# Diegotistical/OptionsLab

Hardware: AMD Instinct MI355X
Metric: MC path-steps/sec (1M paths × 252 steps Euro call); price vs BS |err|/σ (higher is better)
Workload: dtype f32 normals / f64 prices

## Files before the change

### include/olmc.h

```cpp
#ifndef OLMC_H
#define OLMC_H

#include <stdint.h>

#ifdef __cplusplus
extern "C" {
#endif

#define OLMC_ABI_VERSION 6

enum {
    OLMC_OK = 0,
    OLMC_ERR_ARG = 1,
    OLMC_ERR_HIP = 2,
    OLMC_ERR_STATE = 3,
    OLMC_ERR_RCCL = 4
};

enum { OLMC_STREAM_GBM = 0, OLMC_STREAM_HESTON = 1, OLMC_STREAM_JUMP = 2, OLMC_STREAM_KOU = 3 };
enum { OLMC_STREAM_HESTON_QE = 0x48514500 };
enum { OLMC_AVG_ARITHMETIC = 0, OLMC_AVG_GEOMETRIC = 1, OLMC_AVG_ARITHMETIC_FAST = 2 };
#define OLMC_MAX_BATCH 16

typedef struct olmc_stats {
// ... 239 lines not shown
                            const uint32_t* shift, int32_t bits, int antithetic, olmc_stats* out);

int olmc_multi_gpu_european(double S, double K, double T, double r, double sigma, double q, int is_call,
                            int64_t n_paths, int32_t n_steps, uint64_t seed, int antithetic,
                            int n_gpus, olmc_stats* out);
int olmc_multi_gpu_greeks_fd(double S, double K, double T, double r, double sigma, double q, int is_call,
                             int64_t n_paths, int32_t n_steps, uint64_t seed, int second_order,
                             int n_gpus, double* out9, olmc_stats* evals );
int olmc_multi_gpu_european_cv(double S, double K, double T, double r, double sigma, double q, int is_call,
                               int64_t n_paths, int32_t n_steps, uint64_t seed, int antithetic,
                               int n_gpus, olmc_cv_moments* out);
int olmc_multi_gpu_european_qmc(double S, double K, double T, double r, double sigma, double q, int is_call,
                                int64_t n_paths, int32_t dims, const uint32_t* sv, const uint32_t* shift, int32_t bits,
                                int n_gpus, olmc_stats* out);
int olmc_multi_gpu_european_qmc_greeks_fd(double S, double K, double T, double r, double sigma, double q, int is_call,
                                          int64_t n_paths, int32_t dims, const uint32_t* sv, const uint32_t* shift, int32_t bits,
                                          int second_order, int n_gpus, double* out9, olmc_stats* evals );
int olmc_multi_gpu_european_qmc_cv(double S, double K, double T, double r, double sigma, double q, int is_call,
                                   int64_t n_paths, int32_t dims, const uint32_t* sv, const uint32_t* shift, int32_t bits,
                                   int n_gpus, olmc_cv_moments* out);
int olmc_multi_gpu_spans(double* out8);

int olmc_fetch_dev(const double* d_src, int32_t n, void* hip_stream, double* out_host);

int olmc_combine_stats(const olmc_stats* parts, int32_t n_parts, double r, double T, olmc_stats* out);

int olmc_philox_words(uint64_t seed, int64_t path_offset, int64_t n_paths,
                      int32_t block0, int32_t n_blocks, uint32_t stream_tag, uint32_t* out_host);
int olmc_normals(uint64_t seed, int64_t path_offset, int64_t n_paths, int32_t n_steps,
                 float* out_host);

int olmc_profile_enable(int on);
enum { OLMC_TUNE_GRID_CAP = 2, OLMC_TUNE_QMC_BLOCK = 4, OLMC_TUNE_SPLIT_TAIL = 7, OLMC_TUNE_POLL = 8, OLMC_TUNE_SPLIT_SAT = 9,
       OLMC_TUNE_MULTI_LAUNCH = 10, OLMC_TUNE_STAGED_COPY = 11 };
int olmc_tune(int knob, int value);
int olmc_profile_reset(void);
int olmc_kernel_time(int64_t* launches, double* total_ms);

#ifdef __cplusplus
}
#endif
#endif
```

### optionslab_amd/csrc/olmc.hip

```cpp
#include "olmc.h"
#include "olmc_kernels.h"
#include "olmc_job_board.h"

#include <dlfcn.h>
#include <sched.h>
#include <time.h>
#include <hip/hip_ext.h>
#include <rccl/rccl.h>

#include <algorithm>
#include <atomic>
#include <chrono>
#include <climits>
#include <condition_variable>
#include <cmath>
#include <cstdio>
#include <cstdlib>
#include <cstring>
#include <functional>
#include <limits>
#include <mutex>
#include <string>
#include <system_error>
#include <thread>
// ... 26 lines not shown
constexpr int kMaxNV = 2 * OLMC_MAX_BATCH;
constexpr int32_t kMaxGrid = 1 << 18;
constexpr int32_t kMaxGroups = kMaxGrid / kGroupBlocks + 1;
static_assert(kMaxGroups * kMaxNV == kGroupRowsCapacity, "device-side guard must match the group_rows allocation");

struct EventPair {
    hipEvent_t start, stop;
};

struct DeviceCtx {
    int device = -1;
    int cus = 0;
    hipStream_t stream = nullptr;
    struct WsSlot {
        double* block_rows = nullptr;
        size_t cap = 0;
        double* group_rows = nullptr;
        uint32_t* counters = nullptr;
        hipEvent_t done = nullptr;
        bool used = false;
        bool claimed = false;
        hipStream_t owner = nullptr;
        bool shared = false;
    };
    static constexpr int kSlots = 8;
    WsSlot slots[kSlots + 1];
    int next_slot = 0, cur_slot = 0;
    uint64_t* h_flag = nullptr;
    uint64_t* d_flag = nullptr;
    uint64_t seq = 0;
    uint64_t armed = 0;
    double* h_result = nullptr;
    double* d_result = nullptr;
    void* d_bulk = nullptr;
    size_t bulk_bytes = 0;
    void* h_stage[2] = {nullptr, nullptr};
    hipEvent_t stage_landed[2] = {nullptr, nullptr};
    void* d_multi = nullptr;
    void* h_multi = nullptr;
    void* d_h_multi = nullptr;
    int64_t multi_cap = 0;
    size_t multi_bpo = 0;
    size_t multi_off_done = 0, multi_off_opts = 0, multi_off_rows = 0, multi_hoff_out = 0;
    uint32_t* d_sobol = nullptr;
    size_t sobol_words = 0;
    std::vector<uint32_t> sobol_host;
    void* d_bridge = nullptr;
    int32_t bridge_n = 0;
    std::vector<unsigned char> bridge_host;
    double* d_heston_w = nullptr;
    size_t heston_w_bytes = 0;
    bool busy = false;
    std::vector<EventPair> ev_free, ev_pending;
    int64_t prof_launches = 0;
    double prof_ms = 0.0;
};

constexpr int kMaxContexts = 8;

struct DevicePool {
    std::mutex mu;
    std::condition_variable idle;
    std::vector<DeviceCtx*> all;
    int device = -1;
};

std::mutex g_mu;
std::atomic<DevicePool*> g_pool[kMaxDevices] = {};
std::atomic<int> g_default_device{-1};
bool g_profile = false;

int ctx_allocate(DeviceCtx* c) {
    HIP_TRY(hipStreamCreateWithFlags(&c->stream, hipStreamNonBlocking));
    for (auto& sl : c->slots) {
        HIP_TRY(hipMalloc(&sl.group_rows, sizeof(double) * kMaxNV * kMaxGroups));
        HIP_TRY(hipMalloc(&sl.counters, sizeof(uint32_t) * (kMaxGroups + 1) * kCounterStride));
        HIP_TRY(hipMemset(sl.counters, 0, sizeof(uint32_t) * (kMaxGroups + 1) * kCounterStride));
        HIP_TRY(hipEventCreateWithFlags(&sl.done, hipEventDisableTiming));
    }
    HIP_TRY(hipHostMalloc(&c->h_result, sizeof(double) * (kMaxNV + 1 + 15), hipHostMallocMapped));
    HIP_TRY(hipHostGetDevicePointer(reinterpret_cast<void**>(&c->d_result), c->h_result, 0));
    c->h_flag = reinterpret_cast<uint64_t*>(c->h_result + kMaxNV + 8);
    c->d_flag = reinterpret_cast<uint64_t*>(c->d_result + kMaxNV + 8);
    *c->h_flag = 0;
    return OLMC_OK;
}

void ctx_release(DeviceCtx* c) {
    if (c->stream) (void)hipStreamSynchronize(c->stream);
    for (auto& ep : c->ev_pending) { (void)hipEventDestroy(ep.start); (void)hipEventDestroy(ep.stop); }
    for (auto& ep : c->ev_free) { (void)hipEventDestroy(ep.start); (void)hipEventDestroy(ep.stop); }
    if (c->d_bulk) (void)hipFree(c->d_bulk);
    for (int i = 0; i < 2; ++i) {
        if (c->h_stage[i]) (void)hipHostFree(c->h_stage[i]);
        if (c->stage_landed[i]) (void)hipEventDestroy(c->stage_landed[i]);
    }
    if (c->d_multi) (void)hipFree(c->d_multi);
    if (c->h_multi) (void)hipHostFree(c->h_multi);
    if (c->d_sobol) (void)hipFree(c->d_sobol);
    if (c->d_bridge) (void)hipFree(c->d_bridge);
    if (c->d_heston_w) (void)hipFree(c->d_heston_w);
    for (auto& sl : c->slots) {
        if (sl.block_rows) (void)hipFree(sl.block_rows);
        if (sl.group_rows) (void)hipFree(sl.group_rows);
        if (sl.counters) (void)hipFree(sl.counters);
        if (sl.done) (void)hipEventDestroy(sl.done);
    }
    if (c->h_result) (void)hipHostFree(c->h_result);
    if (c->stream) (void)hipStreamDestroy(c->stream);
    delete c;
}

int ctx_create(int device, DeviceCtx** out) {
    int count = 0;
    hipError_t e = hipGetDeviceCount(&count);
    if (e != hipSuccess || count <= 0)
        return fail(OLMC_ERR_HIP, std::string("no HIP device available: ") + hipGetErrorString(e));
    if (device < 0 || device >= count || device >= kMaxDevices)
        return fail(OLMC_ERR_ARG, "device index out of range");
    HIP_TRY(hipSetDevice(device));
    hipDeviceProp_t prop;
    HIP_TRY(hipGetDeviceProperties(&prop, device));
    DeviceCtx* c = new DeviceCtx();
    c->device = device;
    c->cus = prop.multiProcessorCount;
    const int rc = ctx_allocate(c);
    if (rc) {
        ctx_release(c);
        return rc;
    }
    *out = c;
    return OLMC_OK;
}

struct CtxLease {
    DeviceCtx* c = nullptr;
    DevicePool* pool = nullptr;
    CtxLease() = default;
    CtxLease(const CtxLease&) = delete;
    CtxLease& operator=(const CtxLease&) = delete;
    ~CtxLease() { release(); }
// ... 120 lines not shown
        if (err == hipSuccess) err = hipEventRecord(c->stage_landed[slot], c->stream);
        if (err == hipSuccess && i >= 1) {
            const auto t = clock::now();
            err = hipEventSynchronize(c->stage_landed[slot ^ 1]);
            if (i == 1) us_first = us_since(t); else us_events += us_since(t);
            if (err == hipSuccess) landed.store(i, std::memory_order_release);
        }
    }
    {
        const auto t = clock::now();
        if (err == hipSuccess) err = hipEventSynchronize(c->stage_landed[(n_chunks - 1) & 1]);
        us_events += us_since(t);
    }
    if (err == hipSuccess) landed.store(n_chunks, std::memory_order_release);
    else give_up.store(true);
    const auto t_join = clock::now();
    for (std::thread& t : threads) t.join();
    if (trace)
        std::fprintf(stderr, "[olmc copy_to_host] %.1f MB, %lld chunks, %d threads: spawn %.0f us, first chunk landed (kernel + DMA) %.0f us, later event waits %.0f us, "
                             "waits for the copy threads %.0f us, last chunk out + join %.0f us, total %.0f us\n", bytes / 1e6, static_cast<long long>(n_chunks), n_threads,
                     us_spawn, us_first, us_events, us_workers, us_since(t_join), us_since(t_begin));
    if (err != hipSuccess) {
        (void)hipStreamSynchronize(c->stream);
        (void)hipGetLastError();
        return fail(OLMC_ERR_HIP, std::string("copy_to_host: ") + hipGetErrorString(err));
    }
    return OLMC_OK;
}

int g_multi_launch = 0;
int g_grid_cap = 0;
int g_qmc_block = 0;
int g_poll = 0;
int g_split_tail = 0;
int g_split_sat = 0;
#ifdef OLMC_WITH_PROBES
int g_fault_shard = 0;
int g_force_nv = 0;
int g_multi_rehearsal = 0;
#endif

constexpr int32_t kShortPathSteps = 128, kShortPathGrid = 4096;

int32_t grid_for(int64_t n_paths, int32_t n_steps = INT32_MAX) {
    int64_t cap = g_grid_cap > 0 ? std::min<int64_t>(g_grid_cap, kMaxGrid) : kMaxGrid;
    if (g_grid_cap == 0 && n_steps <= kShortPathSteps) cap = kShortPathGrid;
    return static_cast<int32_t>(std::min<int64_t>((n_paths + kBlock - 1) / kBlock, cap));
}

template <typename Kernel>
int resident_workgroups(Kernel kernel) {
    static std::mutex mu;
    static std::vector<std::pair<const void*, int>> cache;
    const void* key = reinterpret_cast<const void*>(kernel);
    std::lock_guard<std::mutex> lock(mu);
    for (const auto& e : cache)
        if (e.first == key) return e.second;
    int nb = 0;
    if (hipOccupancyMaxActiveBlocksPerMultiprocessor(&nb, kernel, kBlock, 0) != hipSuccess || nb < 1) {
        (void)hipGetLastError();
        nb = 1;
    }
    cache.emplace_back(key, nb);
    return nb;
}

// ... 39 lines not shown
            if (!taken.shared) {
                HIP_TRY(hipDeviceSynchronize());
                taken.shared = true;
                taken.used = false;
            }
        }
    }
    DeviceCtx::WsSlot& sl = c->slots[idx];
    c->cur_slot = idx;
    const bool guarded = !own && sl.shared;
    const size_t need = static_cast<size_t>(grid) * nv;
    if (need > sl.cap) {
        if (!guarded) HIP_TRY(hipStreamSynchronize(stream));
        else if (sl.used) HIP_TRY(hipEventSynchronize(sl.done));
        if (sl.block_rows) HIP_TRY(hipFree(sl.block_rows));
        sl.block_rows = nullptr;
        sl.cap = 0;
        const size_t cap = std::max<size_t>(need, size_t(1) << 16);
        HIP_TRY(hipMalloc(&sl.block_rows, sizeof(double) * cap));
        sl.cap = cap;
    }
    if (guarded && sl.used) HIP_TRY(hipStreamWaitEvent(stream, sl.done, 0));
    ws->block_rows = sl.block_rows;
    ws->group_rows = sl.group_rows;
    ws->counters = sl.counters;
    ws->out = d_out;
    ws->tail = tail;
    ws->row_capacity = sl.cap;
#ifdef OLMC_WITH_PROBES
    if (g_force_nv > 0) ws->row_capacity = static_cast<uint64_t>(grid) * g_force_nv;
#endif
    ws->done_flag = nullptr;
    ws->done_value = 0;
    c->armed = 0;
    if (own && d_out == c->d_result && g_poll >= 0) {
        c->armed = ++c->seq;
        ws->done_flag = c->d_flag;
        ws->done_value = c->armed;
    }
    return OLMC_OK;
}

void ws_recover(DeviceCtx* c) {
    c->armed = 0;
    (void)hipDeviceSynchronize();
    (void)hipGetLastError();
    for (auto& sl : c->slots) (void)hipMemset(sl.counters, 0, sizeof(uint32_t) * (kMaxGroups + 1) * kCounterStride);
}

void multi_recover(DeviceCtx* c) {
    c->armed = 0;
    (void)hipDeviceSynchronize();
    (void)hipGetLastError();
    if (c->d_multi) (void)hipMemset(c->d_multi, 0, c->multi_off_opts);
}

int after_launch(DeviceCtx* c, hipStream_t stream) {
    hipError_t e = hipGetLastError();
    if (e != hipSuccess) { ws_recover(c); return fail(OLMC_ERR_HIP, std::string("kernel launch: ") + hipGetErrorString(e)); }
    if (c->cur_slot == DeviceCtx::kSlots || !c->slots[c->cur_slot].shared) return OLMC_OK;
    DeviceCtx::WsSlot& sl = c->slots[c->cur_slot];
    HIP_TRY(hipEventRecord(sl.done, stream));
    sl.used = true;
    return OLMC_OK;
}

int prof_begin(DeviceCtx* c, hipStream_t s, EventPair* ep) {
    if (c->ev_free.empty()) {
        HIP_TRY(hipEventCreate(&ep->start));
        HIP_TRY(hipEventCreate(&ep->stop));
    } else {
        *ep = c->ev_free.back();
        c->ev_free.pop_back();
    }
    HIP_TRY(hipEventRecord(ep->start, s));
    return OLMC_OK;
}
// ... 149 lines not shown
        };
        if (nsets == 1) {
            ContractSet<1> cs;
            cs.c[0] = make_contract(opts[0], n_steps);
            cs.base_mask = 1u; cs.upper_continues_slot0 = 0;
            if (pos) pos[0] = 0;
            launch_european<1, kReduce>(anti, g, st, pr, cs, ws, nullptr, timed);
        } else if (nsets == 8) {
            fused(std::integral_constant<int, 8>{});
        } else {
            fused(std::integral_constant<int, 16>{});
        }
    }, profiled);
}

constexpr int64_t kSpinUs = 200, kYieldUs = 2000, kSleepUs = 20;

struct TimerSlack {
    long old = -1;
    void tighten() {
        if (old >= 0) return;
        old = prctl(PR_GET_TIMERSLACK, 0, 0, 0, 0);
        if (old >= 0 && prctl(PR_SET_TIMERSLACK, 1000UL, 0, 0, 0) != 0) old = -1;
    }
    ~TimerSlack() {
        if (old >= 0) (void)prctl(PR_SET_TIMERSLACK, static_cast<unsigned long>(old), 0, 0, 0);
    }
};

int wait_armed(DeviceCtx* c, hipStream_t s) {
    if (c->armed != 0) {
        const uint64_t want = c->armed;
        c->armed = 0;
        using clock = std::chrono::steady_clock;
        const auto t0 = clock::now();
        bool queried = false;
        int phase = 0;
        TimerSlack slack;
        for (uint32_t spins = 0;; ++spins) {
            if (__atomic_load_n(c->h_flag, __ATOMIC_ACQUIRE) == want) {
                if (queried) (void)hipGetLastError();
                return OLMC_OK;
            }
            if (phase == 0) {
                __builtin_ia32_pause();
                if ((spins & 0x3F) == 0x3F && clock::now() - t0 >= std::chrono::microseconds(kSpinUs)) phase = 1;
                continue;
            }
            if (phase == 1) {
                sched_yield();
                if ((spins & 0xF) == 0xF && clock::now() - t0 >= std::chrono::microseconds(kYieldUs)) phase = 2;
                continue;
            }
            if ((spins & 0x3F) == 0) {
                const hipError_t q = hipStreamQuery(s);
                queried = true;
                if (q == hipSuccess) break;
                if (q != hipErrorNotReady) {
                    ws_recover(c);
                    return fail(OLMC_ERR_HIP, std::string("hipStreamQuery: ") + hipGetErrorString(q));
                }
            }
            slack.tighten();
            const timespec nap{0, kSleepUs * 1000};
            nanosleep(&nap, nullptr);
        }
        (void)hipGetLastError();
    }
    hipError_t e = hipStreamSynchronize(s);
    if (e != hipSuccess) { ws_recover(c); return fail(OLMC_ERR_HIP, std::string("hipStreamSynchronize: ") + hipGetErrorString(e)); }
    return OLMC_OK;
}

int sync_or_recover(DeviceCtx* c, hipStream_t s) {
    if (s != c->stream) c->armed = 0;
    return wait_armed(c, s);
}

int run_batch(const olmc_option* opts, int32_t k, int64_t path_offset, int64_t n_local, int32_t n_steps,
              uint64_t seed, int antithetic, olmc_stats* out, bool prices_only = false) {
    if (!opts || !out) return fail(OLMC_ERR_ARG, "null pointer");
    if (k < 1 || k > OLMC_MAX_BATCH) return fail(OLMC_ERR_ARG, "batch size must be in [1, OLMC_MAX_BATCH]");
    int rc = check_paths(path_offset, n_local, n_steps);
    if (rc) return rc;
    CtxLease lease;
    rc = ctx_lease(&lease);
    if (rc) return rc;
    DeviceCtx* const c = lease.c;
    int pos[OLMC_MAX_BATCH];
    bool lean = prices_only;
    rc = run_batch_device(c, c->stream, opts, k, path_offset, n_local, n_steps, seed, antithetic, c->d_result, -1.0, pos, true, &lean);
    if (rc) return rc;
    finish_set(c->h_result, pos, n_local * (antithetic ? 2 : 1), opts, k, false, lean, out);
    return OLMC_OK;
}

}

namespace { void multi_gpu_release(); }

extern "C" int olmc_abi_version(void) { return OLMC_ABI_VERSION; }

extern "C" const char* olmc_last_error(void) { return t_error.c_str(); }

extern "C" int olmc_init(int device) {
    std::lock_guard<std::mutex> lock(g_mu);
    static const bool env_read = [] {
        const char* p = std::getenv("OLMC_POLL");
        if (p && p[0] == '0') g_poll = -1;
        const char* t = std::getenv("OLMC_SPLIT_TAIL");
        if (t && t[0] == '0') g_split_tail = -1;
        const char* m = std::getenv("OLMC_MULTI_LAUNCH");
        if (m && m[0] == 's') g_multi_launch = -1;
        const char* sc = std::getenv("OLMC_STAGED_COPY");
        if (sc && sc[0] == '0') g_staged_copy = -1;
        return true;
    }();
    (void)env_read;
    if (device < 0 || device >= kMaxDevices) return fail(OLMC_ERR_ARG, "device index out of range");
    if (!g_pool[device].load(std::memory_order_acquire)) {
        DeviceCtx* c = nullptr;
        int rc = ctx_create(device, &c);
        if (rc) return rc;
        DevicePool* pool = new DevicePool();
        pool->device = device;
        pool->all.push_back(c);
        g_pool[device].store(pool, std::memory_order_release);
    } else {
        HIP_TRY(hipSetDevice(device));
    }
    t_device = device;
    if (g_default_device.load() < 0) g_default_device.store(device, std::memory_order_release);
    return OLMC_OK;
}

extern "C" int olmc_shutdown(void) {
    std::lock_guard<std::mutex> lock(g_mu);
    multi_gpu_release();
    for (int d = 0; d < kMaxDevices; ++d) {
        DevicePool* pool = g_pool[d].load();
        if (!pool) continue;
        const bool usable = hipSetDevice(d) == hipSuccess;
        for (DeviceCtx* c : pool->all) {
            if (usable) ctx_release(c);
// ... 33 lines not shown
}

extern "C" int olmc_european_shard(double S, double K, double T, double r, double sigma, double q, int is_call,
                                   int64_t path_offset, int64_t n_local, int32_t n_steps, uint64_t seed,
                                   int antithetic, olmc_stats* out) {
    const olmc_option o = make_option(S, K, T, r, sigma, q, is_call);
    return run_batch(&o, 1, path_offset, n_local, n_steps, seed, antithetic, out);
}

extern "C" int olmc_european_shard_dev(double S, double K, double T, double r, double sigma, double q, int is_call,
                                       int64_t path_offset, int64_t n_local, int32_t n_steps, uint64_t seed,
                                       int antithetic, double* d_triple, void* hip_stream) {
    if (!d_triple) return fail(OLMC_ERR_ARG, "null pointer");
    int rc = check_paths(path_offset, n_local, n_steps);
    if (rc) return rc;
    CtxLease lease;
    rc = ctx_lease(&lease);
    if (rc) return rc;
    DeviceCtx* const c = lease.c;
    hipStream_t s = static_cast<hipStream_t>(hip_stream);
    const olmc_option o = make_option(S, K, T, r, sigma, q, is_call);
    const double n = static_cast<double>(n_local * (antithetic ? 2 : 1));
    return run_batch_device(c, s, &o, 1, path_offset, n_local, n_steps, seed, antithetic, d_triple, n, nullptr, true);
}

namespace {
int fetch_dev(DeviceCtx* c, const double* d_src, int32_t n, hipStream_t s, double* out_host) {
    const uint64_t want = ++c->seq;
    hipLaunchKernelGGL(publish_kernel, dim3(1), dim3(kWave), 0, s, d_src, n, c->d_result, c->d_flag, want);
    HIP_TRY(hipGetLastError());
    int rc = OLMC_OK;
    if (g_poll >= 0) {
        c->armed = want;
        rc = wait_armed(c, s);
    } else {
        hipError_t e = hipStreamSynchronize(s);
        if (e != hipSuccess) rc = fail(OLMC_ERR_HIP, std::string("hipStreamSynchronize: ") + hipGetErrorString(e));
    }
    if (rc) return rc;
    for (int32_t i = 0; i < n; ++i) out_host[i] = c->h_result[i];
    return OLMC_OK;
}
}

extern "C" int olmc_fetch_dev(const double* d_src, int32_t n, void* hip_stream, double* out_host) {
    if (!d_src || !out_host) return fail(OLMC_ERR_ARG, "null pointer");
    if (n < 1 || n > kMaxNV + 1) return fail(OLMC_ERR_ARG, "n must be in [1, 33]");
    CtxLease lease;
    int rc = ctx_lease(&lease);
    if (rc) return rc;
    return fetch_dev(lease.c, d_src, n, static_cast<hipStream_t>(hip_stream), out_host);
}

extern "C" int olmc_european_batch(const olmc_option* opts, int32_t k, int64_t path_offset, int64_t n_local,
                                   int32_t n_steps, uint64_t seed, int antithetic, olmc_stats* out) {
    return run_batch(opts, k, path_offset, n_local, n_steps, seed, antithetic, out);
}

extern "C" int olmc_combine_stats(const olmc_stats* parts, int32_t n_parts, double r, double T, olmc_stats* out) {
    if (!parts || !out || n_parts < 1) return fail(OLMC_ERR_ARG, "bad arguments");
    if (!combine_stats(parts, n_parts, r, T, out)) return fail(OLMC_ERR_ARG, "no samples");
    return OLMC_OK;
}

extern "C" int olmc_european_multi(const olmc_option* opts, const uint32_t* tags, int64_t n_options, int64_t n_paths,
                                   int32_t n_steps, uint64_t seed, int antithetic, olmc_stats* out) {
// ... 16 lines not shown
        HIP_TRY(hipStreamSynchronize(c->stream));
        if (c->d_multi) HIP_TRY(hipFree(c->d_multi));
        if (c->h_multi) HIP_TRY(hipHostFree(c->h_multi));
        c->d_multi = nullptr; c->h_multi = nullptr; c->multi_cap = 0; c->multi_bpo = 0;
        HIP_TRY(hipMalloc(&c->d_multi, b_cnt + b_done + b_opts + b_rows));
        HIP_TRY(hipMemsetAsync(c->d_multi, 0, b_cnt + b_done, c->stream));
        HIP_TRY(hipHostMalloc(&c->h_multi, b_opts + align(sizeof(double) * 2 * cap), hipHostMallocMapped));
        HIP_TRY(hipHostGetDevicePointer(&c->d_h_multi, c->h_multi, 0));
        c->multi_cap = cap;
        c->multi_bpo = bpo_cap;
        c->multi_off_done = b_cnt; c->multi_off_opts = b_cnt + b_done; c->multi_off_rows = b_cnt + b_done + b_opts; c->multi_hoff_out = b_opts;
    }
    char* base = static_cast<char*>(c->d_multi);
    uint32_t* d_cnt = reinterpret_cast<uint32_t*>(base);
    uint32_t* d_done = reinterpret_cast<uint32_t*>(base + c->multi_off_done);
    MultiOption* d_opts = reinterpret_cast<MultiOption*>(base + c->multi_off_opts);
    double* d_rows = reinterpret_cast<double*>(base + c->multi_off_rows);
    MultiOption* h = reinterpret_cast<MultiOption*>(c->h_multi);
    const double* h_out = reinterpret_cast<const double*>(static_cast<char*>(c->h_multi) + c->multi_hoff_out);
    double* d_out = reinterpret_cast<double*>(static_cast<char*>(c->d_h_multi) + c->multi_hoff_out);
    for (int64_t j = 0; j < n_options; ++j) {
        const Contract ct = make_contract(opts[j], n_steps);
        h[j].a = ct.a; h[j].vol = ct.vol; h[j].strike = ct.strike; h[j].sign = ct.sign;
        h[j].tag = tags ? tags[j] : static_cast<uint32_t>(j);
        h[j].pad = 0;
    }
    HIP_TRY(hipMemcpyAsync(d_opts, h, sizeof(MultiOption) * n_options, hipMemcpyHostToDevice, c->stream));
    MultiDone md;
    md.done_count = d_done;
    md.n_total = static_cast<uint32_t>(n_options);
    md.done_flag = nullptr;
    md.done_value = 0;
    c->armed = 0;
    if (g_poll >= 0) {
        c->armed = ++c->seq;
        md.done_flag = c->d_flag;
        md.done_value = c->armed;
    }
    const PathRange pr = make_range(0, n_paths, n_steps, seed);
    EventPair ep{};
    if (g_profile) { rc = prof_begin(c, c->stream, &ep); if (rc) return rc; }
    for (int64_t base_opt = 0; base_opt < n_options; base_opt += 65535) {
        const unsigned ny = static_cast<unsigned>(std::min<int64_t>(65535, n_options - base_opt));
        with_bool(antithetic != 0, [&](auto a) { launch_timed(european_multi_kernel<a>, dim3(bpo, ny), dim3(kBlock), c->stream, nullptr, pr, d_opts, base_opt, d_rows, d_cnt, d_out, md); });
        hipError_t e = hipGetLastError();
        if (e != hipSuccess) {
            multi_recover(c);
            return fail(OLMC_ERR_HIP, std::string("kernel launch: ") + hipGetErrorString(e));
        }
    }
    if (g_profile) { rc = prof_end(c, c->stream, ep); if (rc) { multi_recover(c); return rc; } }
    rc = wait_armed(c, c->stream);
    if (rc) { multi_recover(c); return rc; }
    finish_set(h_out, nullptr, n_paths * (antithetic ? 2 : 1), opts, n_options, false, false, out);
    return OLMC_OK;
}

extern "C" int olmc_contract_layout(const olmc_option* opts, int32_t k, int32_t n_steps, int32_t* nsets_out, int32_t* pos, uint32_t* base_mask,
                                    int32_t* upper_continues_slot0, double* scale16) {
    if (!opts || !nsets_out || !pos || !base_mask || !upper_continues_slot0 || !scale16) return fail(OLMC_ERR_ARG, "null pointer");
    if (k < 2 || k > OLMC_MAX_BATCH) return fail(OLMC_ERR_ARG, "a set has 2 .. OLMC_MAX_BATCH contracts");
    if (n_steps < 1) return fail(OLMC_ERR_ARG, "n_steps must be >= 1");
    contract_layout(opts, k, n_steps, nsets_out, pos, base_mask, upper_continues_slot0, scale16);
    return OLMC_OK;
}

// ... 2273 lines not shown
    hipLaunchKernelGGL(philox_words_kernel, dim3(grid), dim3(256), 0, c->stream, static_cast<uint64_t>(path_offset), n_paths,
                       block0, n_blocks, stream_tag, static_cast<uint32_t>(seed), static_cast<uint32_t>(seed >> 32),
                       static_cast<uint32_t*>(c->d_bulk));
    HIP_TRY(hipGetLastError());
    HIP_TRY(hipMemcpyAsync(out_host, c->d_bulk, bytes, hipMemcpyDeviceToHost, c->stream));
    HIP_TRY(hipStreamSynchronize(c->stream));
    return OLMC_OK;
}

extern "C" int olmc_normals(uint64_t seed, int64_t path_offset, int64_t n_paths, int32_t n_steps, float* out_host) {
    if (!out_host || n_paths < 1 || n_steps < 1 || path_offset < 0) return fail(OLMC_ERR_ARG, "bad arguments");
    CtxLease lease;
    int rc = ctx_lease(&lease);
    if (rc) return rc;
    DeviceCtx* const c = lease.c;
    const size_t bytes = sizeof(float) * static_cast<size_t>(n_paths) * n_steps;
    rc = bulk_reserve(c, bytes);
    if (rc) return rc;
    const int64_t total = n_paths * ((n_steps + 3) / 4);
    const int grid = static_cast<int>(std::min<int64_t>((total + 255) / 256, 4096));
    hipLaunchKernelGGL(normals_kernel, dim3(grid), dim3(256), 0, c->stream, static_cast<uint64_t>(path_offset), n_paths,
                       n_steps, static_cast<uint32_t>(seed), static_cast<uint32_t>(seed >> 32),
                       static_cast<float*>(c->d_bulk));
    HIP_TRY(hipGetLastError());
    HIP_TRY(hipMemcpyAsync(out_host, c->d_bulk, bytes, hipMemcpyDeviceToHost, c->stream));
    HIP_TRY(hipStreamSynchronize(c->stream));
    return OLMC_OK;
}

extern "C" int olmc_tune(int knob, int value) {
    if (knob == OLMC_TUNE_GRID_CAP && value >= 0) { g_grid_cap = value; return OLMC_OK; }
    if (knob == OLMC_TUNE_QMC_BLOCK && value >= -1 && value <= 2) { g_qmc_block = value; return OLMC_OK; }
    if (knob == OLMC_TUNE_POLL && value >= -1 && value <= 0) { g_poll = value; return OLMC_OK; }
    if (knob == OLMC_TUNE_SPLIT_TAIL && value >= -1 && value <= 0) { g_split_tail = value; return OLMC_OK; }
    if (knob == OLMC_TUNE_SPLIT_SAT && value >= 0 && value <= 16) { g_split_sat = value; return OLMC_OK; }
    if (knob == OLMC_TUNE_MULTI_LAUNCH && value >= -1 && value <= 0) { g_multi_launch = value; return OLMC_OK; }
    if (knob == OLMC_TUNE_STAGED_COPY && value >= -1 && value <= 0) { g_staged_copy = value; return OLMC_OK; }
    return fail(OLMC_ERR_ARG, "unknown tuning knob or value");
}

namespace {
template <typename Fn>
int with_all_contexts(Fn fn) {
    int dev = t_device >= 0 ? t_device : g_default_device.load(std::memory_order_acquire);
    if (dev < 0) {
        int rc = olmc_init(0);
        if (rc) return rc;
        dev = t_device;
    }
    DevicePool* pool = g_pool[dev].load(std::memory_order_acquire);
    if (!pool) return fail(OLMC_ERR_STATE, "device not initialised (call olmc_init)");
    HIP_TRY(hipSetDevice(dev));
    std::vector<DeviceCtx*> mine;
    {
        std::unique_lock<std::mutex> lock(pool->mu);
        pool->idle.wait(lock, [&] { return std::none_of(pool->all.begin(), pool->all.end(), [](const DeviceCtx* c) { return c->busy; }); });
        mine = pool->all;
        for (DeviceCtx* c : mine) c->busy = true;
    }
    int rc = OLMC_OK;
    for (DeviceCtx* c : mine) {
        const int r = fn(c);
        if (r && !rc) rc = r;
    }
    {
        std::lock_guard<std::mutex> lock(pool->mu);
// ... 50 lines not shown
```

### optionslab_amd/csrc/olmc_host_math.h

```cpp
#ifndef OLMC_HOST_MATH_H
#define OLMC_HOST_MATH_H

#include "olmc.h"

#include <algorithm>
#include <cmath>
#include <cstdint>
#include <cstring>

namespace olmc {

struct Contract {
    double a;
    double vol;
    double strike;
    double sign;
    double scale;
    double neg_sign_strike;
    double sign_scale;
};

template <int NSETS>
struct ContractSet {
    Contract c[NSETS];
// ... 291 lines not shown
        if (!geometric && n_groups > 0 && same_bits(as->vol[0], vol) && !same_bits(as->drift[0], drift)) {
            int d = 0;
            while (d < n_riders && !same_bits(rider_drift[d], drift)) ++d;
            if (d == n_riders) {
                if (n_riders == kAsianGroups - kAsianRealGroups) return "more drift-only bumps than the fused Asian Greeks kernel carries";
                rider_drift[d] = drift;
                as->rate_step[d] = drift - as->drift[0];
                ++n_riders;
            }
            as->group[i] = kAsianRealGroups + d;
            continue;
        }
        int g = 0;
        while (g < n_groups && !(same_bits(as->drift[g], drift) && same_bits(as->vol[g], vol))) ++g;
        if (g == n_groups) {
            if (n_groups == real_slots) return "more distinct path recursions than the fused Asian Greeks kernel carries";
            as->drift[g] = drift;
            as->vol[g] = vol;
            ++n_groups;
        }
        as->group[i] = g;
    }
    for (int g = n_groups; g < kAsianGroups; ++g) { as->drift[g] = as->drift[0]; as->vol[g] = as->vol[0]; }
    for (int g = 0; g < kAsianGroups; ++g) {
        as->drift[g] = as->drift[g] * unit;
        as->vol[g] = as->vol[g] * kZScale * unit;
    }
    as->strike = K;
    as->sign = is_call ? 1.0 : -1.0;
    as->inv_steps = 1.0 / n_steps;
    return nullptr;
}

inline void shard_range(int64_t n_paths, int rank, int n_ranks, int64_t* lo, int64_t* count) {
    const int64_t a = n_paths * rank / n_ranks, b = n_paths * (rank + 1) / n_ranks;
    *lo = a;
    *count = b - a;
}

constexpr int64_t kQmcShardAlign = 512, kQmcShardMinPoints = 4096;
inline void qmc_shard_range(int64_t n_points, int rank, int n_ranks, int64_t* lo, int64_t* count) {
    if (n_points / n_ranks < kQmcShardMinPoints) return shard_range(n_points, rank, n_ranks, lo, count);
    const int64_t a = n_points * rank / n_ranks / kQmcShardAlign * kQmcShardAlign;
    const int64_t b = rank + 1 == n_ranks ? n_points : n_points * (rank + 1) / n_ranks / kQmcShardAlign * kQmcShardAlign;
    *lo = a;
    *count = b - a;
}

}

#endif
```

### optionslab_amd/csrc/olmc_kernels.h

```cpp
#pragma once
#include <type_traits>
#include <hip/hip_runtime.h>
#include <stdint.h>

#include "olmc_host_math.h"

namespace olmc {

constexpr int kBlock = 256;
constexpr int kWave = 64;
constexpr int kWavesPerBlock = kBlock / kWave;

constexpr uint32_t kPhiloxM0 = 0xD2511F53u;
constexpr uint32_t kPhiloxM1 = 0xCD9E8D57u;
constexpr uint32_t kPhiloxW0 = 0x9E3779B9u;
constexpr uint32_t kPhiloxW1 = 0xBB67AE85u;

struct Words4 {
    uint32_t x0, x1, x2, x3;
};

__device__ __forceinline__ uint32_t xor3(uint32_t a, uint32_t b, uint32_t c) {
    return __builtin_amdgcn_bitop3_b32(a, b, c, 0x96);
}
// ... 131 lines not shown
                s = __builtin_fmaf(z_cos, kInvSqrt2F, s);
            }
            q += static_cast<double>(s);
        }
        acc += q;
    }
    return acc;
}

__device__ __forceinline__ double path_normal_sum(uint32_t g_lo, uint32_t g_hi, int32_t n_steps, uint32_t k0, uint32_t k1,
                                                  uint32_t tag = 0u) {
    return path_normal_quarters(g_lo, g_hi, n_steps, 0, 4, k0, k1, tag) * kPairZScale;
}

__device__ __forceinline__ double wave_sum(double v) {
#pragma unroll
    for (int off = kWave / 2; off > 0; off >>= 1) v += __shfl_down(v, off, kWave);
    return v;
}

constexpr int kGroupBlocks = 256;
constexpr int kGroupRowsCapacity = ((1 << 18) / kGroupBlocks + 1) * 32;
constexpr int kCounterStride = 64;

struct ReduceWs {
    double* block_rows;
    double* group_rows;
    uint32_t* counters;
    double* out;
    double tail;
    uint64_t row_capacity;
    uint64_t* done_flag;
    uint64_t done_value;
};

__device__ __forceinline__ void signal_done(const ReduceWs& ws) {
    if (ws.done_flag == nullptr) return;
    __builtin_amdgcn_fence(__ATOMIC_RELEASE, "");
    if (threadIdx.x == 0) __hip_atomic_store(ws.done_flag, ws.done_value, __ATOMIC_RELAXED, __HIP_MEMORY_SCOPE_SYSTEM);
}

#ifndef OLMC_AGENT_ACQUIRE
#define OLMC_AGENT_ACQUIRE 1
#endif
#if !OLMC_AGENT_ACQUIRE && defined(__HIP_DEVICE_COMPILE__) && !defined(__gfx942__) && !defined(__gfx950__)
#error "OLMC_AGENT_ACQUIRE=0 relies on gfx942 / gfx950 cache behaviour (sc1 rows are L2-served): build this target with the acquire"
#endif
__device__ __forceinline__ void acquire_rows() {
#if OLMC_AGENT_ACQUIRE
    __builtin_amdgcn_fence(__ATOMIC_ACQUIRE, "agent");
#else
    __builtin_amdgcn_fence(__ATOMIC_ACQUIRE, "wavefront");
#endif
}

__device__ __forceinline__ void store_sc1(double* p, double v) {
    __hip_atomic_store(p, v, __ATOMIC_RELAXED, __HIP_MEMORY_SCOPE_AGENT);
}
__device__ __forceinline__ double load_sc1(const double* p) {
    return __hip_atomic_load(p, __ATOMIC_RELAXED, __HIP_MEMORY_SCOPE_AGENT);
}

template <int NV>
__device__ __forceinline__ double wave_rows_sum(const double* src, int32_t rows) {
    constexpr int NVP = NV <= 2 ? 2 : NV <= 8 ? 8 : NV <= 16 ? 16 : 32;
    constexpr int SUBS = kWave / NVP;
    const int lane = threadIdx.x & (kWave - 1);
    const int c = lane % NVP, sub = lane / NVP;
    double v = 0.0;
    if (c < NV) {
        constexpr int kBatch = 8;
        for (int32_t row = sub; row < rows; row += SUBS * kBatch) {
            double t[kBatch];
#pragma unroll
            for (int j = 0; j < kBatch; ++j) {
                const int32_t rj = row + j * SUBS;
                t[j] = rj < rows ? load_sc1(src + static_cast<size_t>(rj) * NV + c) : 0.0;
            }
#pragma unroll
            for (int j = 0; j < kBatch; ++j) v += t[j];
        }
    }
#pragma unroll
    for (int off = kWave / 2; off >= NVP; off >>= 1) v += __shfl_down(v, off, kWave);
    return v;
}

struct NoEpilogue {
    __device__ __forceinline__ void operator()(double) const {}
};

template <int NV, typename Epilogue = NoEpilogue>
__device__ __forceinline__ void grid_reduce(double v, const ReduceWs& ws, Epilogue done = Epilogue()) {
    const int lane = threadIdx.x;
    const int32_t n_blocks = static_cast<int32_t>(gridDim.x);
    const int32_t n_groups = (n_blocks + kGroupBlocks - 1) / kGroupBlocks;
    const int32_t group = static_cast<int32_t>(blockIdx.x) / kGroupBlocks;
    const int32_t group_size = min(kGroupBlocks, n_blocks - group * kGroupBlocks);

    if (static_cast<uint64_t>(n_blocks) * NV > ws.row_capacity || n_groups * NV > kGroupRowsCapacity) {
        if (blockIdx.x == 0) {
            if (lane < NV) ws.out[lane] = __builtin_nan("");
            signal_done(ws);
        }
        return;
    }
    if (lane < NV) store_sc1(ws.block_rows + static_cast<size_t>(blockIdx.x) * NV + lane, v);
    asm volatile("s_waitcnt vmcnt(0)" ::: "memory");
    uint32_t ticket = 0;
    if (lane == 0) ticket = __hip_atomic_fetch_add(ws.counters + static_cast<size_t>(group) * kCounterStride, 1u, __ATOMIC_RELAXED, __HIP_MEMORY_SCOPE_AGENT);
    ticket = __builtin_amdgcn_readfirstlane(ticket);
    if (ticket != static_cast<uint32_t>(group_size - 1)) return;

    acquire_rows();
    const double g = wave_rows_sum<NV>(ws.block_rows + static_cast<size_t>(group) * kGroupBlocks * NV, group_size);
    if (n_groups == 1) {
        if (lane < NV) ws.out[lane] = g;
        if (lane == 0) {
            if (ws.tail >= 0.0) ws.out[NV] = ws.tail;
            __hip_atomic_store(ws.counters, 0u, __ATOMIC_RELAXED, __HIP_MEMORY_SCOPE_AGENT);
        }
        done(g);
        signal_done(ws);
        return;
    }
    if (lane < NV) store_sc1(ws.group_rows + static_cast<size_t>(group) * NV + lane, g);
    asm volatile("s_waitcnt vmcnt(0)" ::: "memory");
    if (lane == 0) {
        __hip_atomic_store(ws.counters + static_cast<size_t>(group) * kCounterStride, 0u, __ATOMIC_RELAXED, __HIP_MEMORY_SCOPE_AGENT);
        ticket = __hip_atomic_fetch_add(ws.counters + static_cast<size_t>(n_groups) * kCounterStride, 1u, __ATOMIC_RELAXED, __HIP_MEMORY_SCOPE_AGENT);
    }
    ticket = __builtin_amdgcn_readfirstlane(ticket);
    if (ticket != static_cast<uint32_t>(n_groups - 1)) return;

    acquire_rows();
    const double total = wave_rows_sum<NV>(ws.group_rows, n_groups);
    if (lane < NV) ws.out[lane] = total;
    if (lane == 0) {
        if (ws.tail >= 0.0) ws.out[NV] = ws.tail;
        __hip_atomic_store(ws.counters + static_cast<size_t>(n_groups) * kCounterStride, 0u, __ATOMIC_RELAXED, __HIP_MEMORY_SCOPE_AGENT);
    }
    done(total);
    signal_done(ws);
}

template <int NV>
__device__ __forceinline__ double workgroup_rows_sum(const double* src, int32_t rows, double* part ) {
    constexpr int NVP = NV <= 8 ? 8 : NV <= 16 ? 16 : 32;
    constexpr int SUBS = kBlock / NVP;
    const int c = threadIdx.x % NVP, sub = threadIdx.x / NVP;
    double v = 0.0;
    if (c < NV) {
        constexpr int kBatch = NVP >= 16 ? 16 : 8;
        for (int32_t row = sub; row < rows; row += SUBS * kBatch) {
            double t[kBatch];
#pragma unroll
            for (int j = 0; j < kBatch; ++j) {
                const int32_t rj = row + j * SUBS;
                t[j] = rj < rows ? load_sc1(src + static_cast<size_t>(rj) * NV + c) : 0.0;
            }
#pragma unroll
            for (int j = 0; j < kBatch; ++j) v += t[j];
        }
    }
    part[threadIdx.x] = v;
    __syncthreads();
    double total = 0.0;
    if (threadIdx.x < NV) {
#pragma unroll
        for (int k = 0; k < SUBS; ++k) total += part[k * NVP + threadIdx.x];
    }
    __syncthreads();
    return total;
}

template <int NV, typename Epilogue = NoEpilogue>
__device__ __forceinline__ void grid_reduce_workgroup(double v, const ReduceWs& ws, Epilogue done = Epilogue()) {
    __shared__ double part[kBlock];
    __shared__ uint32_t last;
    const int t = threadIdx.x;
    const bool wave0 = t < kWave;
    const int32_t n_blocks = static_cast<int32_t>(gridDim.x);
    const int32_t n_groups = (n_blocks + kGroupBlocks - 1) / kGroupBlocks;
    const int32_t group = static_cast<int32_t>(blockIdx.x) / kGroupBlocks;
    const int32_t group_size = min(kGroupBlocks, n_blocks - group * kGroupBlocks);

    if (static_cast<uint64_t>(n_blocks) * NV > ws.row_capacity || n_groups * NV > kGroupRowsCapacity) {
        if (blockIdx.x == 0 && wave0) {
            if (t < NV) ws.out[t] = __builtin_nan("");
            signal_done(ws);
        }
        return;
    }
    if (wave0) {
        if (t < NV) store_sc1(ws.block_rows + static_cast<size_t>(blockIdx.x) * NV + t, v);
        asm volatile("s_waitcnt vmcnt(0)" ::: "memory");
        if (t == 0) last = __hip_atomic_fetch_add(ws.counters + static_cast<size_t>(group) * kCounterStride, 1u, __ATOMIC_RELAXED, __HIP_MEMORY_SCOPE_AGENT) ==
                           static_cast<uint32_t>(group_size - 1);
    }
    __syncthreads();
    if (!last) return;

    acquire_rows();
    const double g = workgroup_rows_sum<NV>(ws.block_rows + static_cast<size_t>(group) * kGroupBlocks * NV, group_size, part);
    if (n_groups == 1) {
        if (wave0) {
            if (t < NV) ws.out[t] = g;
            if (t == 0) {
                if (ws.tail >= 0.0) ws.out[NV] = ws.tail;
                __hip_atomic_store(ws.counters, 0u, __ATOMIC_RELAXED, __HIP_MEMORY_SCOPE_AGENT);
            }
            done(g);
            signal_done(ws);
        }
        return;
    }
    if (wave0) {
        if (t < NV) store_sc1(ws.group_rows + static_cast<size_t>(group) * NV + t, g);
        asm volatile("s_waitcnt vmcnt(0)" ::: "memory");
        if (t == 0) {
            __hip_atomic_store(ws.counters + static_cast<size_t>(group) * kCounterStride, 0u, __ATOMIC_RELAXED, __HIP_MEMORY_SCOPE_AGENT);
            last = __hip_atomic_fetch_add(ws.counters + static_cast<size_t>(n_groups) * kCounterStride, 1u, __ATOMIC_RELAXED, __HIP_MEMORY_SCOPE_AGENT) ==
                   static_cast<uint32_t>(n_groups - 1);
        }
    }
    __syncthreads();
    if (!last) return;

    acquire_rows();
    const double total = workgroup_rows_sum<NV>(ws.group_rows, n_groups, part);
    if (wave0) {
        if (t < NV) ws.out[t] = total;
        if (t == 0) {
            if (ws.tail >= 0.0) ws.out[NV] = ws.tail;
            __hip_atomic_store(ws.counters + static_cast<size_t>(n_groups) * kCounterStride, 0u, __ATOMIC_RELAXED, __HIP_MEMORY_SCOPE_AGENT);
        }
        done(total);
        signal_done(ws);
    }
}

__device__ __forceinline__ uint32_t dbl_lo(double x) { return static_cast<uint32_t>(__double_as_longlong(x)); }
__device__ __forceinline__ uint32_t dbl_hi(double x) { return static_cast<uint32_t>(static_cast<uint64_t>(__double_as_longlong(x)) >> 32); }
__device__ __forceinline__ double dbl_of(uint32_t lo, uint32_t hi) {
    return __longlong_as_double(static_cast<long long>((static_cast<uint64_t>(hi) << 32) | lo));
}

struct SumOp {
    __device__ __forceinline__ double operator()(double a, double b) const { return a + b; }
};

template <int OFF, typename Op = SumOp>
__device__ __forceinline__ double swap_add(double a, double b) {
    static_assert(OFF == 32 || OFF == 16, "permlane swaps exist for half-waves and rows");
    if constexpr (OFF == 32) {
        const auto lo = __builtin_amdgcn_permlane32_swap(dbl_lo(a), dbl_lo(b), false, false);
        const auto hi = __builtin_amdgcn_permlane32_swap(dbl_hi(a), dbl_hi(b), false, false);
        return Op()(dbl_of(lo[0], hi[0]), dbl_of(lo[1], hi[1]));
    } else {
        const auto lo = __builtin_amdgcn_permlane16_swap(dbl_lo(a), dbl_lo(b), false, false);
        const auto hi = __builtin_amdgcn_permlane16_swap(dbl_hi(a), dbl_hi(b), false, false);
        return Op()(dbl_of(lo[0], hi[0]), dbl_of(lo[1], hi[1]));
    }
}

template <int P, int OFF = kWave / 2, typename Op = SumOp>
__device__ __forceinline__ void wave_transpose_reduce(double (&v)[P]) {
    if constexpr (P > 1) {
        constexpr int H = P / 2;
        double kept[H];
        if constexpr (OFF >= 16) {
// ... 3388 lines not shown
```

Before: 2453 billion.

## Finish multi-group grid reduction on host from mapped per-group rows

When a launch has several reduction groups and the epilogue only observes, each group's last block writes its partial row to host-mapped memory and publishes a per-group sequence word. The host poller then sums the rows itself instead of waiting for a final cross-group pass on the device. The release fence in signal_done is also replaced by a vmcnt wait, with result stores made system-scope atomics. This shortens the device-side tail of the reduction but adds PCIe-visible stores, host-side summation, and subtle memory-ordering risk.

```diff
diff --git a/include/olmc.h b/include/olmc.h
--- a/include/olmc.h
+++ b/include/olmc.h
@@ -295,7 +295,7 @@
 
 int olmc_profile_enable(int on);
 enum { OLMC_TUNE_GRID_CAP = 2, OLMC_TUNE_QMC_BLOCK = 4, OLMC_TUNE_SPLIT_TAIL = 7, OLMC_TUNE_POLL = 8, OLMC_TUNE_SPLIT_SAT = 9,
-       OLMC_TUNE_MULTI_LAUNCH = 10, OLMC_TUNE_STAGED_COPY = 11 };
+       OLMC_TUNE_MULTI_LAUNCH = 10, OLMC_TUNE_STAGED_COPY = 11, OLMC_TUNE_HOST_FINISH = 12 };
 int olmc_tune(int knob, int value);
 int olmc_profile_reset(void);
 int olmc_kernel_time(int64_t* launches, double* total_ms);
diff --git a/optionslab_amd/csrc/olmc.hip b/optionslab_amd/csrc/olmc.hip
--- a/optionslab_amd/csrc/olmc.hip
+++ b/optionslab_amd/csrc/olmc.hip
@@ -82,6 +82,13 @@
     uint64_t armed = 0;
     double* h_result = nullptr;
     double* d_result = nullptr;
+    double* h_rows = nullptr;
+    double* d_rows = nullptr;
+    uint64_t* h_seq = nullptr;
+    uint64_t* d_seq = nullptr;
+    int32_t armed_groups = 0;
+    int armed_nv = 0;
+    double armed_tail = -1.0;
     void* d_bulk = nullptr;
     size_t bulk_bytes = 0;
     void* h_stage[2] = {nullptr, nullptr};
@@ -133,6 +140,13 @@
     c->h_flag = reinterpret_cast<uint64_t*>(c->h_result + kMaxNV + 8);
     c->d_flag = reinterpret_cast<uint64_t*>(c->d_result + kMaxNV + 8);
     *c->h_flag = 0;
+    constexpr size_t kRowsBytes = sizeof(double) * kMaxNV * kMaxGroups, kSeqBytes = sizeof(uint64_t) * kMaxGroups;
+    static_assert(kRowsBytes % 64 == 0, "the words start on a cache line of their own");
+    HIP_TRY(hipHostMalloc(&c->h_rows, kRowsBytes + kSeqBytes, hipHostMallocMapped));
+    HIP_TRY(hipHostGetDevicePointer(reinterpret_cast<void**>(&c->d_rows), c->h_rows, 0));
+    c->h_seq = reinterpret_cast<uint64_t*>(c->h_rows + kMaxNV * kMaxGroups);
+    c->d_seq = reinterpret_cast<uint64_t*>(c->d_rows + kMaxNV * kMaxGroups);
+    std::memset(c->h_rows, 0, kRowsBytes + kSeqBytes);
     return OLMC_OK;
 }
 
@@ -157,6 +171,7 @@
         if (sl.done) (void)hipEventDestroy(sl.done);
     }
     if (c->h_result) (void)hipHostFree(c->h_result);
+    if (c->h_rows) (void)hipHostFree(c->h_rows);
     if (c->stream) (void)hipStreamDestroy(c->stream);
     delete c;
 }
@@ -343,6 +358,7 @@
 int g_grid_cap = 0;
 int g_qmc_block = 0;
 int g_poll = 0;
+int g_host_finish = 1;
 int g_split_tail = 0;
 int g_split_sat = 0;
 #ifdef OLMC_WITH_PROBES
@@ -448,17 +464,29 @@
 #endif
     ws->done_flag = nullptr;
     ws->done_value = 0;
+    ws->host_rows = nullptr;
+    ws->host_seq = nullptr;
     c->armed = 0;
+    c->armed_groups = 0;
     if (own && d_out == c->d_result && g_poll >= 0) {
         c->armed = ++c->seq;
         ws->done_flag = c->d_flag;
         ws->done_value = c->armed;
+        const int32_t n_groups = (grid + kGroupBlocks - 1) / kGroupBlocks;
+        if (g_host_finish > 0 && n_groups >= 2 && n_groups <= kMaxGroups && nv >= 1 && nv <= kMaxNV) {
+            ws->host_rows = c->d_rows;
+            ws->host_seq = c->d_seq;
+            c->armed_groups = n_groups;
+            c->armed_nv = nv;
+            c->armed_tail = tail;
+        }
     }
     return OLMC_OK;
 }
 
 void ws_recover(DeviceCtx* c) {
     c->armed = 0;
+    c->armed_groups = 0;
     (void)hipDeviceSynchronize();
     (void)hipGetLastError();
     for (auto& sl : c->slots) (void)hipMemset(sl.counters, 0, sizeof(uint32_t) * (kMaxGroups + 1) * kCounterStride);
@@ -674,12 +702,22 @@
     if (c->armed != 0) {
         const uint64_t want = c->armed;
         c->armed = 0;
+        const int32_t n_groups = c->armed_groups;
+        c->armed_groups = 0;
+        int32_t seen = 0;
         using clock = std::chrono::steady_clock;
         const auto t0 = clock::now();
-        bool queried = false;
+        bool queried = false, retired_short = false;
         int phase = 0;
         TimerSlack slack;
         for (uint32_t spins = 0;; ++spins) {
+            while (seen < n_groups && __atomic_load_n(c->h_seq + seen, __ATOMIC_ACQUIRE) == want) ++seen;
+            if (seen == n_groups && n_groups > 0) {
+                host_rows_sum(c->h_rows, n_groups, c->armed_nv, c->h_result);
+                if (c->armed_tail >= 0.0) c->h_result[c->armed_nv] = c->armed_tail;
+                if (queried) (void)hipGetLastError();
+                return OLMC_OK;
+            }
             if (__atomic_load_n(c->h_flag, __ATOMIC_ACQUIRE) == want) {
                 if (queried) (void)hipGetLastError();
                 return OLMC_OK;
@@ -697,7 +735,10 @@
             if ((spins & 0x3F) == 0) {
                 const hipError_t q = hipStreamQuery(s);
                 queried = true;
-                if (q == hipSuccess) break;
+                if (q == hipSuccess) {
+                    retired_short = n_groups > 0;
+                    break;
+                }
                 if (q != hipErrorNotReady) {
                     ws_recover(c);
                     return fail(OLMC_ERR_HIP, std::string("hipStreamQuery: ") + hipGetErrorString(q));
@@ -708,6 +749,18 @@
             nanosleep(&nap, nullptr);
         }
         (void)hipGetLastError();
+        if (retired_short) {
+            while (seen < n_groups && __atomic_load_n(c->h_seq + seen, __ATOMIC_ACQUIRE) == want) ++seen;
+            if (seen == n_groups) {
+                host_rows_sum(c->h_rows, n_groups, c->armed_nv, c->h_result);
+                if (c->armed_tail >= 0.0) c->h_result[c->armed_nv] = c->armed_tail;
+                return OLMC_OK;
+            }
+            if (__atomic_load_n(c->h_flag, __ATOMIC_ACQUIRE) != want) {
+                ws_recover(c);
+                return fail(OLMC_ERR_HIP, "the launch retired without delivering its group rows");
+            }
+        }
     }
     hipError_t e = hipStreamSynchronize(s);
     if (e != hipSuccess) { ws_recover(c); return fail(OLMC_ERR_HIP, std::string("hipStreamSynchronize: ") + hipGetErrorString(e)); }
@@ -752,6 +805,8 @@
         if (p && p[0] == '0') g_poll = -1;
         const char* t = std::getenv("OLMC_SPLIT_TAIL");
         if (t && t[0] == '0') g_split_tail = -1;
+        const char* hf = std::getenv("OLMC_HOST_FINISH");
+        if (hf && hf[0] == '0') g_host_finish = 0;
         const char* m = std::getenv("OLMC_MULTI_LAUNCH");
         if (m && m[0] == 's') g_multi_launch = -1;
         const char* sc = std::getenv("OLMC_STAGED_COPY");
@@ -851,6 +906,7 @@
     int rc = OLMC_OK;
     if (g_poll >= 0) {
         c->armed = want;
+        c->armed_groups = 0;
         rc = wait_armed(c, s);
     } else {
         hipError_t e = hipStreamSynchronize(s);
@@ -933,6 +989,7 @@
     md.done_flag = nullptr;
     md.done_value = 0;
     c->armed = 0;
+    c->armed_groups = 0;
     if (g_poll >= 0) {
         c->armed = ++c->seq;
         md.done_flag = c->d_flag;
@@ -3272,6 +3329,7 @@
     if (knob == OLMC_TUNE_GRID_CAP && value >= 0) { g_grid_cap = value; return OLMC_OK; }
     if (knob == OLMC_TUNE_QMC_BLOCK && value >= -1 && value <= 2) { g_qmc_block = value; return OLMC_OK; }
     if (knob == OLMC_TUNE_POLL && value >= -1 && value <= 0) { g_poll = value; return OLMC_OK; }
+    if (knob == OLMC_TUNE_HOST_FINISH && value >= 0 && value <= 1) { g_host_finish = value; return OLMC_OK; }
     if (knob == OLMC_TUNE_SPLIT_TAIL && value >= -1 && value <= 0) { g_split_tail = value; return OLMC_OK; }
     if (knob == OLMC_TUNE_SPLIT_SAT && value >= 0 && value <= 16) { g_split_sat = value; return OLMC_OK; }
     if (knob == OLMC_TUNE_MULTI_LAUNCH && value >= -1 && value <= 0) { g_multi_launch = value; return OLMC_OK; }
diff --git a/optionslab_amd/csrc/olmc_host_math.h b/optionslab_amd/csrc/olmc_host_math.h
--- a/optionslab_amd/csrc/olmc_host_math.h
+++ b/optionslab_amd/csrc/olmc_host_math.h
@@ -347,6 +347,34 @@
     return nullptr;
 }
 
+inline void host_rows_sum(const double* src, int32_t rows, int nv, double* out) {
+    const bool wave = nv <= 2;
+    const int nvp = nv <= 2 ? 2 : nv <= 8 ? 8 : nv <= 16 ? 16 : 32;
+    const int lanes = wave ? 64 : 256, subs = lanes / nvp, batch = (!wave && nvp >= 16) ? 16 : 8;
+    for (int c = 0; c < nv; ++c) {
+        double part[128];
+        for (int sub = 0; sub < subs; ++sub) {
+            double v = 0.0;
+            for (int32_t row = sub; row < rows; row += subs * batch)
+                for (int j = 0; j < batch; ++j) {
+                    const int64_t rj = static_cast<int64_t>(row) + static_cast<int64_t>(j) * subs;
+                    const double t = rj < rows ? src[rj * nv + c] : 0.0;
+                    v = v + t;
+                }
+            part[sub] = v;
+        }
+        if (wave) {
+            for (int off = subs / 2; off >= 1; off >>= 1)
+                for (int sub = 0; sub < off; ++sub) part[sub] = part[sub] + part[sub + off];
+            out[c] = part[0];
+        } else {
+            double total = 0.0;
+            for (int k = 0; k < subs; ++k) total = total + part[k];
+            out[c] = total;
+        }
+    }
+}
+
 inline void shard_range(int64_t n_paths, int rank, int n_ranks, int64_t* lo, int64_t* count) {
     const int64_t a = n_paths * rank / n_ranks, b = n_paths * (rank + 1) / n_ranks;
     *lo = a;
diff --git a/optionslab_amd/csrc/olmc_kernels.h b/optionslab_amd/csrc/olmc_kernels.h
--- a/optionslab_amd/csrc/olmc_kernels.h
+++ b/optionslab_amd/csrc/olmc_kernels.h
@@ -187,11 +187,27 @@
     uint64_t row_capacity;
     uint64_t* done_flag;
     uint64_t done_value;
-};
-
+    double* host_rows;
+    uint64_t* host_seq;
+};
+
+template <typename E, typename = void>
+struct epilogue_observes_only { static constexpr bool value = false; };
+template <typename E>
+struct epilogue_observes_only<E, typename std::enable_if<E::kObserverOnly>::type> { static constexpr bool value = true; };
+
+__device__ __forceinline__ void store_sys(double* p, double v) {
+    __hip_atomic_store(p, v, __ATOMIC_RELAXED, __HIP_MEMORY_SCOPE_SYSTEM);
+}
+
+#ifndef OLMC_SIGNAL_FENCE
+#define OLMC_SIGNAL_FENCE 0
+#endif
+template <bool FENCED = false>
 __device__ __forceinline__ void signal_done(const ReduceWs& ws) {
     if (ws.done_flag == nullptr) return;
-    __builtin_amdgcn_fence(__ATOMIC_RELEASE, "");
+    if constexpr (FENCED || OLMC_SIGNAL_FENCE) __builtin_amdgcn_fence(__ATOMIC_RELEASE, "");
+    else asm volatile("s_waitcnt vmcnt(0)" ::: "memory");
     if (threadIdx.x == 0) __hip_atomic_store(ws.done_flag, ws.done_value, __ATOMIC_RELAXED, __HIP_MEMORY_SCOPE_SYSTEM);
 }
 
@@ -242,11 +258,13 @@
 }
 
 struct NoEpilogue {
+    static constexpr bool kObserverOnly = true;
     __device__ __forceinline__ void operator()(double) const {}
 };
 
 template <int NV, typename Epilogue = NoEpilogue>
 __device__ __forceinline__ void grid_reduce(double v, const ReduceWs& ws, Epilogue done = Epilogue()) {
+    constexpr bool kObserver = epilogue_observes_only<Epilogue>::value, kFenced = !kObserver;
     const int lane = threadIdx.x;
     const int32_t n_blocks = static_cast<int32_t>(gridDim.x);
     const int32_t n_groups = (n_blocks + kGroupBlocks - 1) / kGroupBlocks;
@@ -255,7 +273,7 @@
 
     if (static_cast<uint64_t>(n_blocks) * NV > ws.row_capacity || n_groups * NV > kGroupRowsCapacity) {
         if (blockIdx.x == 0) {
-            if (lane < NV) ws.out[lane] = __builtin_nan("");
+            if (lane < NV) store_sys(ws.out + lane, __builtin_nan(""));
             signal_done(ws);
         }
         return;
@@ -270,14 +288,26 @@
     acquire_rows();
     const double g = wave_rows_sum<NV>(ws.block_rows + static_cast<size_t>(group) * kGroupBlocks * NV, group_size);
     if (n_groups == 1) {
-        if (lane < NV) ws.out[lane] = g;
+        if (lane < NV) store_sys(ws.out + lane, g);
         if (lane == 0) {
-            if (ws.tail >= 0.0) ws.out[NV] = ws.tail;
+            if (ws.tail >= 0.0) store_sys(ws.out + NV, ws.tail);
             __hip_atomic_store(ws.counters, 0u, __ATOMIC_RELAXED, __HIP_MEMORY_SCOPE_AGENT);
         }
         done(g);
-        signal_done(ws);
+        signal_done<kFenced>(ws);
         return;
+    }
+    if constexpr (kObserver) {
+        if (ws.host_rows != nullptr) {
+            if (lane < NV) store_sys(ws.host_rows + static_cast<size_t>(group) * NV + lane, g);
+            asm volatile("s_waitcnt vmcnt(0)" ::: "memory");
+            if (lane == 0) {
+                __hip_atomic_store(ws.counters + static_cast<size_t>(group) * kCounterStride, 0u, __ATOMIC_RELAXED, __HIP_MEMORY_SCOPE_AGENT);
+                __hip_atomic_store(ws.host_seq + group, ws.done_value, __ATOMIC_RELAXED, __HIP_MEMORY_SCOPE_SYSTEM);
+            }
+            done(g);
+            return;
+        }
     }
     if (lane < NV) store_sc1(ws.group_rows + static_cast<size_t>(group) * NV + lane, g);
     asm volatile("s_waitcnt vmcnt(0)" ::: "memory");
@@ -290,13 +320,13 @@
 
     acquire_rows();
     const double total = wave_rows_sum<NV>(ws.group_rows, n_groups);
-    if (lane < NV) ws.out[lane] = total;
+    if (lane < NV) store_sys(ws.out + lane, total);
     if (lane == 0) {
-        if (ws.tail >= 0.0) ws.out[NV] = ws.tail;
+        if (ws.tail >= 0.0) store_sys(ws.out + NV, ws.tail);
         __hip_atomic_store(ws.counters + static_cast<size_t>(n_groups) * kCounterStride, 0u, __ATOMIC_RELAXED, __HIP_MEMORY_SCOPE_AGENT);
     }
     done(total);
-    signal_done(ws);
+    signal_done<kFenced>(ws);
 }
 
 template <int NV>
@@ -333,6 +363,7 @@
 __device__ __forceinline__ void grid_reduce_workgroup(double v, const ReduceWs& ws, Epilogue done = Epilogue()) {
     __shared__ double part[kBlock];
     __shared__ uint32_t last;
+    constexpr bool kObserver = epilogue_observes_only<Epilogue>::value, kFenced = !kObserver;
     const int t = threadIdx.x;
     const bool wave0 = t < kWave;
     const int32_t n_blocks = static_cast<int32_t>(gridDim.x);
@@ -342,7 +373,7 @@
 
     if (static_cast<uint64_t>(n_blocks) * NV > ws.row_capacity || n_groups * NV > kGroupRowsCapacity) {
         if (blockIdx.x == 0 && wave0) {
-            if (t < NV) ws.out[t] = __builtin_nan("");
+            if (t < NV) store_sys(ws.out + t, __builtin_nan(""));
             signal_done(ws);
         }
         return;
@@ -360,15 +391,29 @@
     const double g = workgroup_rows_sum<NV>(ws.block_rows + static_cast<size_t>(group) * kGroupBlocks * NV, group_size, part);
     if (n_groups == 1) {
         if (wave0) {
-            if (t < NV) ws.out[t] = g;
+            if (t < NV) store_sys(ws.out + t, g);
             if (t == 0) {
-                if (ws.tail >= 0.0) ws.out[NV] = ws.tail;
+                if (ws.tail >= 0.0) store_sys(ws.out + NV, ws.tail);
                 __hip_atomic_store(ws.counters, 0u, __ATOMIC_RELAXED, __HIP_MEMORY_SCOPE_AGENT);
             }
             done(g);
-            signal_done(ws);
+            signal_done<kFenced>(ws);
         }
         return;
+    }
+    if constexpr (kObserver) {
+        if (ws.host_rows != nullptr) {
+            if (wave0) {
+                if (t < NV) store_sys(ws.host_rows + static_cast<size_t>(group) * NV + t, g);
+                asm volatile("s_waitcnt vmcnt(0)" ::: "memory");
+                if (t == 0) {
+                    __hip_atomic_store(ws.counters + static_cast<size_t>(group) * kCounterStride, 0u, __ATOMIC_RELAXED, __HIP_MEMORY_SCOPE_AGENT);
+                    __hip_atomic_store(ws.host_seq + group, ws.done_value, __ATOMIC_RELAXED, __HIP_MEMORY_SCOPE_SYSTEM);
+                }
+                done(g);
+            }
+            return;
+        }
     }
     if (wave0) {
         if (t < NV) store_sc1(ws.group_rows + static_cast<size_t>(group) * NV + t, g);
@@ -385,13 +430,13 @@
     acquire_rows();
     const double total = workgroup_rows_sum<NV>(ws.group_rows, n_groups, part);
     if (wave0) {
-        if (t < NV) ws.out[t] = total;
+        if (t < NV) store_sys(ws.out + t, total);
         if (t == 0) {
-            if (ws.tail >= 0.0) ws.out[NV] = ws.tail;
+            if (ws.tail >= 0.0) store_sys(ws.out + NV, ws.tail);
             __hip_atomic_store(ws.counters + static_cast<size_t>(n_groups) * kCounterStride, 0u, __ATOMIC_RELAXED, __HIP_MEMORY_SCOPE_AGENT);
         }
         done(total);
-        signal_done(ws);
+        signal_done<kFenced>(ws);
     }
 }
 
```

Result: no change. 2466 billion, median of 6 (+0.5%).
